# lambdaclass/lambdaworks_cairo_prover

Hardware: AMD Instinct MI355X
Metric: stark252_ntt_field_ops_per_s (higher is better)
Workload: dtype u256 mod p (8 x u32 Montgomery limbs); 1 GPU; Stark252 forward NTT 2^22, natural order in/out, one vector per GPU (BASELINE configs[1]); log_n=22, parallelism=replicas x1 (column sharding, no collective), self_warmup_steps=930

## Files before the change

include/stark252_hip.h:

```cpp
#ifndef STARK252_HIP_H
#define STARK252_HIP_H
#include <stddef.h>
#include <stdint.h>

#ifdef __cplusplus
extern "C" {
#endif

enum {
    SP_OK = 0,
    SP_E_INVALID_ARG = -1,
    SP_E_NO_DEVICE = -2,
    SP_E_HIP = -3,
    SP_E_ALLOC = -4,
    SP_E_STATE = -5,
    SP_E_ZERO_INVERSE = -6,
    SP_E_UNSUPPORTED = -7,
    SP_E_PROGRAM = -8
};

typedef enum { SP_FE_MONT_LIMBS = 0, SP_FE_CANON_BE = 1 } sp_fe_encoding;

typedef struct {
    uint8_t blowup_factor;
// ... 16 lines not shown

typedef int (*sp_allgather_fn)(void* user, const void* send_dev, void* recv_dev, uint64_t bytes_per_rank);

const char* sp_version(void);
#define SP_ABI_VERSION 7
int sp_abi_version(void);
uint64_t sp_air_desc_size(void);
const char* sp_last_error(void);
int sp_device_count(int* count_out);
int sp_host_cpus(int* count_out);
int sp_host_cpu_budget(int* budget_out, int* ranks_out);
int sp_host_bind_to_device(int device, int* node_out);

int sp_ctx_create(sp_ctx** ctx_out, const sp_config* cfg);
void sp_ctx_destroy(sp_ctx* ctx);

int sp_set_collective(sp_ctx* ctx, int world, int rank, sp_allgather_fn fn, void* user);
int sp_comm_unique_id(uint8_t id_out[128]);
int sp_comm_init_rccl(sp_ctx* ctx, const uint8_t id[128], int world, int rank);
typedef int (*sp_allgather_async_fn)(void* user, const void* send_dev, void* recv_dev, uint64_t bytes_per_rank, void* hip_stream);
int sp_set_collective_async(sp_ctx* ctx, sp_allgather_async_fn fn);
int sp_comm_init_null(sp_ctx* ctx, int world, int rank);
typedef int (*sp_alltoall_fn)(void* user, const void* send_dev, void* recv_dev, uint64_t bytes_per_pair);
int sp_set_alltoall(sp_ctx* ctx, sp_alltoall_fn fn);
typedef int (*sp_alltoall_async_fn)(void* user, const void* send_dev, void* recv_dev, uint64_t bytes_per_pair, void* hip_stream);
int sp_set_alltoall_async(sp_ctx* ctx, sp_alltoall_async_fn fn);
int sp_comm_stats(sp_ctx* ctx, uint64_t out[6]);
int sp_comm_time_ms(sp_ctx* ctx, double out[2]);
int sp_comm_selftest(sp_ctx* ctx, uint64_t bytes_per_block);
#define SP_LINK_MEASURED_MARGIN 1.25
int sp_comm_measure(sp_ctx* ctx, uint64_t bytes_per_rank, double out[6]);
int sp_model_shard_interpolation(double link_gbs_per_direction, uint32_t groups, uint32_t log2_rows);
enum { SP_OPT_FRI_SHARD_MIN_LOG = 1, SP_OPT_SHARD_INTERPOLATION = 2, SP_OPT_UPLOAD_THREADS = 3, SP_OPT_MERKLE_BACKEND = 4, SP_OPT_MERKLE_ONE_COLUMN_ROWS = 5,
       SP_OPT_DEVICE_TRACE = 6, SP_OPT_LINK_GBS = 7, SP_OPT_HOST_RANKS = 8 };
enum { SP_MERKLE_KECCAK256 = 0, SP_MERKLE_POSEIDON = 1 };
int sp_set_option(sp_ctx* ctx, int key, int64_t value);


int sp_ntt(sp_ctx* ctx, uint8_t* data, uint64_t n, int inverse, const uint8_t* coset);

int sp_ntt_dev(sp_ctx* ctx, void* data_dev, uint64_t n, uint32_t batch, int inverse, const uint8_t* coset);

int sp_lde(sp_ctx* ctx, const uint8_t* coeffs, uint64_t n, uint32_t cols, uint32_t blowup, const uint8_t* coset,
           uint8_t* out);

int sp_merkle_build(sp_ctx* ctx, const uint8_t* leaves, uint64_t n_leaves, uint32_t fe_per_leaf,
                    uint8_t root_out[32], uint8_t* nodes_out);

int sp_merkle_build_dev(sp_ctx* ctx, const void* cols_dev, uint64_t n_leaves, uint32_t fe_per_leaf, uint64_t col_stride,
                        void* nodes_dev);

int sp_batch_inverse(sp_ctx* ctx, uint8_t* data, uint64_t n);
int sp_fe_mul(sp_ctx* ctx, const uint8_t* a, const uint8_t* b, uint64_t n, uint8_t* out);

int sp_fe_to_device(int fe_encoding, const uint8_t* in, uint64_t n, uint8_t* out_device_layout);
int sp_fe_from_device(int fe_encoding, const uint8_t* in_device_layout, uint64_t n, uint8_t* out);

int sp_sync(sp_ctx* ctx);
int sp_last_kernel_ms(sp_ctx* ctx, float* ms_out);
int sp_timer_start(sp_ctx* ctx);
int sp_timer_stop(sp_ctx* ctx, float* ms_out);

typedef struct {
    uint8_t pc_init[32], ap_init[32], fp_init[32], pc_final[32], ap_final[32];
    uint16_t range_check_min, range_check_max;
    uint32_t n_segments;
    const uint8_t* segment_types;
// ... 244 lines not shown
```

lambdaworks_cairo_prover_amd/api.py:

```python
import ctypes
from dataclasses import dataclass

import numpy as np

from . import _lib
from ._lib import (SP_FE_CANON_BE, SP_FE_MONT_LIMBS, CairoPublicInputsC, ConfigC, ProofOptionsC, SpError, check)

__all__ = ["ProofOptions", "Context", "CairoRun", "generate_prover_args_fibonacci", "SpError", "P", "felts_to_bytes",
           "bytes_to_felts", "SP_FE_CANON_BE", "SP_FE_MONT_LIMBS"]

P = 2**251 + 17 * 2**192 + 1


def felts_to_bytes(values):
    return np.frombuffer(b"".join(int(v).to_bytes(32, "big") for v in values), dtype=np.uint8).reshape(-1, 32).copy()


def bytes_to_felts(arr):
    b = np.ascontiguousarray(arr, dtype=np.uint8).tobytes()
    return [int.from_bytes(b[i:i + 32], "big") for i in range(0, len(b), 32)]


@dataclass
class ProofOptions:
# ... 719 lines not shown
    check(self._lib.sp_comm_selftest(self._h, ctypes.c_uint64(bytes_per_block)))


def _ctx_comm_measure(self, bytes_per_rank=64 << 20):
    out = (ctypes.c_double * 6)()
    check(self._lib.sp_comm_measure(self._h, ctypes.c_uint64(int(bytes_per_rank)), out))
    return {"allgather_ms": out[0], "allgather_gbs_per_link": out[1], "alltoall_ms": out[2], "alltoall_gbs_per_link": out[3],
            "bytes_per_rank": int(out[4]), "world": int(out[5])}


LINK_MEASURED_MARGIN = 1.25


def model_shard_interpolation(link_gbs, groups, log2_rows):
    lib = _lib.load()
    lib.sp_model_shard_interpolation.argtypes = [ctypes.c_double, ctypes.c_uint32, ctypes.c_uint32]
    return int(lib.sp_model_shard_interpolation(float(link_gbs), int(groups), int(log2_rows)))


def _ctx_comm_time_ms(self):
    out = (ctypes.c_double * 2)()
    check(self._lib.sp_comm_time_ms(self._h, out))
    return out[0], out[1]


def _ctx_comm_stats(self):
    out = (ctypes.c_uint64 * 6)()
    check(self._lib.sp_comm_stats(self._h, out))
    return {"world": out[0], "allgather_calls": out[1], "allgather_bytes": out[2], "alltoall_calls": out[3],
            "alltoall_bytes": out[4], "received_bytes": out[5]}


SP_OPT_FRI_SHARD_MIN_LOG, SP_OPT_SHARD_INTERPOLATION, SP_OPT_UPLOAD_THREADS, SP_OPT_MERKLE_BACKEND, SP_OPT_MERKLE_ONE_COLUMN_ROWS, SP_OPT_DEVICE_TRACE, SP_OPT_LINK_GBS, SP_OPT_HOST_RANKS = 1, 2, 3, 4, 5, 6, 7, 8
SP_MERKLE_KECCAK256, SP_MERKLE_POSEIDON = 0, 1
SP_PREWARM_KERNELS, SP_PREWARM_CLOCKS, SP_PREWARM_HOST_ROWS, SP_PREWARM_ALL = 1, 2, 4, 7


def _ctx_set_option(self, key, value):
    check(self._lib.sp_set_option(self._h, int(key), ctypes.c_int64(int(value))))


def _ctx_init_rccl(self, group=None):
    import torch
    import torch.distributed as dist
    world, rank = dist.get_world_size(group), dist.get_rank(group)
    idb = (ctypes.c_uint8 * 128)()
    if rank == 0:
        check(self._lib.sp_comm_unique_id(idb))
    obj = [bytes(idb)]
    dist.broadcast_object_list(obj, src=0, group=group)
    check(self._lib.sp_comm_init_rccl(self._h, obj[0], world, rank))


Context.set_collective = _ctx_set_collective
Context.init_rccl = _ctx_init_rccl
Context.init_null = _ctx_init_null
Context.set_collective_async = _ctx_set_collective_async
Context.comm_stats = _ctx_comm_stats
Context.comm_selftest = _ctx_comm_selftest
Context.comm_measure = _ctx_comm_measure
Context.comm_time_ms = _ctx_comm_time_ms
Context.set_option = _ctx_set_option
__all__ += ["cairo_verify", "proof_file_bytes", "proof_file_verify", "StagedAllGather", "StagedAsyncAllGather", "shard_global_index", "interleave_shards",
            "SP_OPT_FRI_SHARD_MIN_LOG", "SP_OPT_SHARD_INTERPOLATION", "SP_OPT_UPLOAD_THREADS", "SP_OPT_MERKLE_BACKEND", "SP_OPT_MERKLE_ONE_COLUMN_ROWS", "SP_OPT_DEVICE_TRACE", "SP_OPT_LINK_GBS", "SP_OPT_HOST_RANKS", "host_cpu_budget", "last_error", "model_shard_interpolation",
            "SP_MERKLE_KECCAK256", "SP_MERKLE_POSEIDON", "poseidon_host", "host_bind_to_device",
            "SP_PREWARM_KERNELS", "SP_PREWARM_CLOCKS", "SP_PREWARM_HOST_ROWS", "SP_PREWARM_ALL"]
```

lambdaworks_cairo_prover_amd/csrc/capi_dev.cpp:

```cpp
#include "ctx.h"
#include "cairo_host.h"
#include <rccl/rccl.h>
#include <chrono>
#include <cstdlib>
#include <algorithm>
#include <cstring>
#include <vector>

namespace sp { int air_periodic_tables(hipStream_t st, NttEngine& ntt, fe* vals, fe* ws, fe* tab, uint32_t cnt, uint32_t logp, uint32_t logn, uint32_t logb, const fe& h); }
namespace sp { int air_stride_class_tables(hipStream_t st, NttEngine& ntt, fe* u, fe* z, uint32_t logs, uint32_t offset, uint32_t logn, uint32_t logb, const fe& h); }
using namespace sp;

namespace {
struct DevBuf {
    void* p = nullptr;
    ~DevBuf() { if (p) (void)hipFree(p); }
    int alloc(size_t bytes) {
        if (hipMalloc(&p, bytes ? bytes : 1) != hipSuccess) { sp_set_error("hipMalloc failed (" + std::to_string(bytes) + " bytes)"); p = nullptr; return SP_E_ALLOC; }
        return SP_OK;
    }
    template <class T> T* as() { return reinterpret_cast<T*>(p); }
};
}

// ... 101 lines not shown
int sp_set_option(sp_ctx* c, int key, int64_t value) {
    if (!c) return SP_E_INVALID_ARG;
    switch (key) {
        case SP_OPT_FRI_SHARD_MIN_LOG:
            if (value < 1 || value > 40) return SP_E_INVALID_ARG;
            c->opt_fri_shard_min_log = (uint32_t)value;
            break;
        case SP_OPT_SHARD_INTERPOLATION:
            if (value < 0 || value > 2) return SP_E_INVALID_ARG;
            c->opt_shard_interpolation = (int)value;
            break;
        case SP_OPT_LINK_GBS:
            if (value < 1 || value > 10000) return SP_E_INVALID_ARG;
            c->opt_link_gbs = (double)value;
            c->opt_link_gbs_explicit = true;
            break;
        case SP_OPT_UPLOAD_THREADS:
            if (value < 1 || value > 128) return SP_E_INVALID_ARG;
            c->opt_upload_threads = (uint32_t)value;
            break;
        case SP_OPT_MERKLE_BACKEND:
            if (value != SP_MERKLE_KECCAK256 && value != SP_MERKLE_POSEIDON) return SP_E_INVALID_ARG;
            c->opt_merkle_backend = (int)value;
            break;
        case SP_OPT_HOST_RANKS:
            if (value < 0 || value > 1024) return SP_E_INVALID_ARG;
            sp::set_host_ranks((unsigned)value);
            return SP_OK;
        case SP_OPT_DEVICE_TRACE:
            c->opt_device_trace = value != 0;
            return SP_OK;
        case SP_OPT_MERKLE_ONE_COLUMN_ROWS:
            c->opt_merkle_one_column_rows = value != 0;
            return SP_OK;
        default: sp_set_error("sp_set_option: unknown key"); return SP_E_INVALID_ARG;
    }
    delete c->prover_state_deleter_holder;
    c->prover_state_deleter_holder = nullptr;
    return SP_OK;
}

namespace {
struct RcclComm : public sp_deletable {
    ncclComm_t comm = nullptr;
    hipStream_t stream = nullptr;
    int world = 1;
    ~RcclComm() override { if (comm) (void)ncclCommDestroy(comm); }
};
int rccl_allgather(void* user, const void* send, void* recv, uint64_t bytes) {
    RcclComm* rc = static_cast<RcclComm*>(user);
    if (ncclAllGather(send, recv, bytes, ncclUint8, rc->comm, rc->stream) != ncclSuccess) return -1;
    if (hipStreamSynchronize(rc->stream) != hipSuccess) return -2;
    return 0;
}
int rccl_allgather_async(void* user, const void* send, void* recv, uint64_t bytes, void* stream) {
    RcclComm* rc = static_cast<RcclComm*>(user);
    return ncclAllGather(send, recv, bytes, ncclUint8, rc->comm, static_cast<hipStream_t>(stream)) == ncclSuccess ? 0 : -1;
}
int rccl_alltoall_async(void* user, const void* send, void* recv, uint64_t bytes, void* stream) {
    RcclComm* rc = static_cast<RcclComm*>(user);
    hipStream_t st = static_cast<hipStream_t>(stream);
    const uint8_t* s = static_cast<const uint8_t*>(send);
    uint8_t* r = static_cast<uint8_t*>(recv);
    if (ncclGroupStart() != ncclSuccess) return -1;
    int rcode = 0;
    for (int peer = 0; peer < rc->world && rcode == 0; ++peer) {
// ... 524 lines not shown
```

lambdaworks_cairo_prover_amd/csrc/ntt.h:

```cpp
#pragma once
#include "common.h"
#include <map>
#include <vector>

namespace sp {

constexpr int NTT_TILE_LOG = 10;
constexpr int NTT_THREADS = 256;
constexpr int NTT_MAX_CONTIG_LOG = NTT_TILE_LOG;
constexpr int NTT_STRIDED_G_LOG = 2;
constexpr int NTT_MAX_STRIDED_LOG = NTT_TILE_LOG - NTT_STRIDED_G_LOG;

struct NttPassArgs {
    const fe* src;
    fe* dst;
    uint64_t src_vec_stride, dst_vec_stride;
    const fe* small_tw;
    const fe* big_tw;
    const fe* post_table;
    const fe* scalar;
    uint32_t logM;
    uint32_t logL;
    uint32_t s, r, g;
    uint32_t log_expand;
    uint32_t tw_shift, tw_low;
    uint32_t coset_count, shard_log;
    uint64_t src_coset_stride, dst_coset_stride;
    uint32_t weak_out;
    uint32_t stage_tw;
    uint32_t radix4;
    uint32_t batch;
    uint32_t xcd_map;
};

enum NttLoadMode { NTT_LOAD_INPLACE = 0, NTT_LOAD_GATHER_BITREV = 1, NTT_LOAD_EXPAND = 2 };
enum NttStoreMode { NTT_STORE_INPLACE = 0, NTT_STORE_SCATTER_BITREV = 1 };

class NttEngine {
  public:
    explicit NttEngine(hipStream_t stream) : stream_(stream) {}
    ~NttEngine();
    int roots(int k, const fe** out);
    int stage_tables(int k, const fe** out);
    int inv_roots_small(int k, const fe** out);

    int dit_bitrev_to_natural(fe* data, int k, uint32_t batch, uint64_t stride);
    int dif_natural_to_bitrev_inverse(fe* data, int k, uint32_t batch, uint64_t stride, const fe* post_table, const fe* src = nullptr);
    int forward_natural(const fe* src, fe* dst, int k, uint32_t batch, uint64_t src_stride, uint64_t dst_stride, fe* final_dst = nullptr);
    int inverse_natural(fe* data, fe* tmp, int k, uint32_t batch, uint64_t stride);
    int lde_from_bitrev(const fe* coeffs, fe* dst, int k, int logb, uint32_t batch, uint64_t src_stride, uint64_t dst_stride,
                        int shard_log = 0, int shard_rank = 0);
    int lde_coset_major(const fe* coeffs, fe* dst, int k, int logb, uint32_t batch, uint64_t src_stride, uint64_t dst_stride,
                        int shard_log = 0, int shard_rank = 0);

    int scale_by_powers(fe* data, uint64_t n, uint32_t batch, uint64_t stride, const fe& base, const fe* c);

    hipStream_t stream() const { return stream_; }

  private:
    int launch_pass(bool dif, int load_mode, int store_mode, const NttPassArgs& a, uint32_t batch);
    hipStream_t stream_;
    int transform_twiddles(int k, NttPassArgs* a);
    std::map<int, fe*> roots_;
    std::vector<fe*> pyramids_;
    int pyramid_log_ = -1;
    std::map<int, fe*> inv_small_;
    fe* d_scalar_ = nullptr;
};

fe host_primitive_root(int k);

}
```

lambdaworks_cairo_prover_amd/csrc/ntt.hip:

```cpp
#include "ntt.h"
#include <algorithm>

#ifndef SP_NTT_STAGE_TW
#define SP_NTT_STAGE_TW 1
#endif

namespace sp {

__device__ __forceinline__ fe ld_fe(const fe* p) {
    const uint4* q = reinterpret_cast<const uint4*>(p);
    uint4 lo = q[0], hi = q[1];
    fe r;
    r.v[0] = lo.x; r.v[1] = lo.y; r.v[2] = lo.z; r.v[3] = lo.w;
    r.v[4] = hi.x; r.v[5] = hi.y; r.v[6] = hi.z; r.v[7] = hi.w;
    return r;
}
__device__ __forceinline__ void st_fe(fe* p, const fe& a) {
    uint4* q = reinterpret_cast<uint4*>(p);
    q[0] = make_uint4(a.v[0], a.v[1], a.v[2], a.v[3]);
    q[1] = make_uint4(a.v[4], a.v[5], a.v[6], a.v[7]);
}
__device__ __forceinline__ fe lds_ld(const uint4* lo, const uint4* hi, uint32_t i) {
    uint4 a = lo[i], b = hi[i];
    fe r;
    r.v[0] = a.x; r.v[1] = a.y; r.v[2] = a.z; r.v[3] = a.w;
    r.v[4] = b.x; r.v[5] = b.y; r.v[6] = b.z; r.v[7] = b.w;
    return r;
}
__device__ __forceinline__ void lds_st(uint4* lo, uint4* hi, uint32_t i, const fe& a) {
    lo[i] = make_uint4(a.v[0], a.v[1], a.v[2], a.v[3]);
    hi[i] = make_uint4(a.v[4], a.v[5], a.v[6], a.v[7]);
}
__device__ __forceinline__ uint32_t bitrev(uint32_t x, uint32_t bits) { return bits ? (__brev(x) >> (32 - bits)) : 0u; }

template <bool DIF, int LOADM, int STOREM, bool CONTIG, bool GTW>
__global__ void __launch_bounds__(NTT_THREADS) ntt_pass_kernel(NttPassArgs a) {
    extern __shared__ __attribute__((aligned(16))) uint4 smem[];
#ifndef SP_NTT_PRIO
#define SP_NTT_PRIO 1
#endif
    if (SP_NTT_PRIO & 1) __builtin_amdgcn_s_setprio(3);
    const uint32_t r = a.r, g = a.g;
    const uint32_t s = a.s;
    const uint32_t R = 1u << r, G = 1u << g, TILE = R << g;
    constexpr bool GLOBAL_TW = GTW;
    static_assert(GTW || CONTIG, "strided passes stage the twiddles of their own butterflies");
    uint4* Llo = smem;
    uint4* Lhi = smem + TILE;
    uint4* Twl = smem + 2 * TILE;
    uint4* Twh = Twl + (GLOBAL_TW ? (CONTIG ? R : (a.radix4 ? (TILE >> 2) : (TILE >> 1))) : (R >> 1));
    const uint32_t tid = threadIdx.x;
    uint32_t tile, vec;
    if (a.xcd_map) {
        const uint32_t xcd = blockIdx.x & 7u, slot = blockIdx.x >> 3;
        const uint32_t tg = slot / a.batch;
        vec = slot - tg * a.batch;
        tile = (tg << 3) | xcd;
    } else {
        tile = blockIdx.x / a.batch;
        vec = blockIdx.x - tile * a.batch;
    }
    uint32_t tw_low = a.tw_low;
    const fe* src;
    fe* dst;
    if (a.coset_count) {
        const uint32_t v = vec / a.coset_count, cl = vec - v * a.coset_count;
        src = a.src + (uint64_t)v * a.src_vec_stride + (uint64_t)cl * a.src_coset_stride;
        dst = a.dst + (uint64_t)v * a.dst_vec_stride + (uint64_t)cl * a.dst_coset_stride;
        tw_low |= cl << a.shard_log;
    } else {
        src = a.src + (uint64_t)vec * a.src_vec_stride;
        dst = a.dst + (uint64_t)vec * a.dst_vec_stride;
    }
    const uint32_t logM = a.logM;
    const uint32_t logL = a.logL;
    const uint32_t sg = s + a.tw_shift;

    uint32_t lo0 = 0, hi = 0;
    if (!CONTIG) {
        uint32_t lo_tiles = 1u << (s - g);
        lo0 = (tile & (lo_tiles - 1)) << g;
        hi = tile >> (s - g);
    }
    auto global_tw = [&](uint32_t jm1, uint32_t i, uint32_t gl) -> fe {
        const uint32_t col = ((lo0 + gl) << a.tw_shift) | tw_low;
        const uint32_t x = (i << sg) + col, h = 1u << (sg + jm1);
        const bool pyr = SP_NTT_STAGE_TW && a.stage_tw;
        const uint32_t sh = pyr ? 0u : logM - sg - jm1 - 1u, off = pyr ? h : 0u;
        if (!DIF) return ld_fe(a.big_tw + off + (x << sh));
        if (x == 0) return fe_neg_one();
        return ld_fe(a.big_tw + off + ((h - x) << sh));
    };
    constexpr int BPT = (1 << (NTT_TILE_LOG - 1)) / NTT_THREADS;
    fe tw_last[(GLOBAL_TW && !CONTIG) ? BPT : 1];
    fe tw_pen;
    if (GLOBAL_TW && CONTIG) {
        for (uint32_t x = tid; x + 1 < R; x += NTT_THREADS) {
            const uint32_t y = x + 1u, jm1 = 31u - __clz(y);
            lds_st(Twl, Twh, x, global_tw(jm1, y - (1u << jm1), 0u));
        }
    } else if (GLOBAL_TW) {
        if (r >= 1) {
#pragma unroll
            for (int q = 0; q < BPT; ++q) {
                const uint32_t b = tid + q * (a.radix4 ? (TILE >> 2) : (uint32_t)NTT_THREADS);
                if (b < (TILE >> 1)) tw_last[q] = global_tw(r - 1, b >> g, b & (G - 1));
            }
            if (a.radix4 && r >= 2 && tid < (TILE >> 2)) tw_pen = global_tw(r - 2, tid >> g, tid & (G - 1));
            const uint32_t cnt = (a.radix4 ? (TILE >> 2) : (TILE >> 1)) - G;
            fe tmp[BPT];
#pragma unroll
            for (int q = 0; q < BPT; ++q) {
                const uint32_t x = tid + q * NTT_THREADS;
                if (x < cnt) {
                    const uint32_t y = (x >> g) + 1u;
                    const uint32_t jm1 = 31u - __clz(y);
                    tmp[q] = global_tw(jm1, y - (1u << jm1), x & (G - 1));
                }
            }
#pragma unroll
            for (int q = 0; q < BPT; ++q) {
                const uint32_t x = tid + q * NTT_THREADS;
                if (x < cnt) lds_st(Twl, Twh, x, tmp[q]);
            }
        }
    } else {
        for (uint32_t i = tid; i < (R >> 1); i += NTT_THREADS) lds_st(Twl, Twh, i, ld_fe(a.small_tw + i));
    }
    auto position = [&](uint32_t t, uint32_t gl) -> uint32_t {
        if (CONTIG) {
            if (LOADM == NTT_LOAD_GATHER_BITREV || STOREM == NTT_STORE_SCATTER_BITREV)
                return (bitrev((tile << g) + gl, logL - r) << r) + t;
            return (tile << (r + g)) + (gl << r) + t;
        }
        return (hi << (s + r)) + (t << s) + lo0 + gl;
    };
    auto lidx = [&](uint32_t t, uint32_t gl) -> uint32_t { return CONTIG ? (gl << r) + t : (t << g) + gl; };

    constexpr int LU = 4;
    for (uint32_t e0 = tid; e0 < TILE; e0 += NTT_THREADS * LU) {
        fe xs[LU];
        uint32_t li[LU];
#pragma unroll
        for (int q = 0; q < LU; ++q) {
            const uint32_t e = e0 + q * NTT_THREADS;
            if (e >= TILE) continue;
            uint32_t t, gl;
            if (CONTIG && LOADM == NTT_LOAD_INPLACE) {
                t = e & (R - 1); gl = e >> r;
                xs[q] = ld_fe(src + position(t, gl));
            } else if (CONTIG) {
                gl = e & (G - 1); t = e >> g;
                uint32_t sidx = (bitrev(t, r) << (logL - r)) + (tile << g) + gl;
                xs[q] = ld_fe(src + sidx);
            } else {
                gl = e & (G - 1); t = e >> g;
                uint32_t pos = position(t, gl);
                if (LOADM == NTT_LOAD_EXPAND) xs[q] = ld_fe(src + (pos >> s));
                else xs[q] = ld_fe(src + pos);
            }
            li[q] = lidx(t, gl);
        }
#pragma unroll
        for (int q = 0; q < LU; ++q)
            if (e0 + q * NTT_THREADS < TILE) lds_st(Llo, Lhi, li[q], xs[q]);
    }
    if (SP_NTT_PRIO & 1) __builtin_amdgcn_s_setprio(0);
    __syncthreads();

// ... 114 lines not shown
                    const uint32_t q = half;
                    st_fe(dst + position(t0, gl), a.weak_out ? fe_reduce_lazy_2p(y0) : fe_canonical_lazy(y0));
                    st_fe(dst + position(t0 + q, gl), a.weak_out ? fe_reduce_lazy_2p(y1) : fe_canonical_lazy(y1));
                    st_fe(dst + position(t0 + 2 * q, gl), a.weak_out ? fe_reduce_lazy_2p(y2) : fe_canonical_lazy(y2));
                    st_fe(dst + position(t0 + 3 * q, gl), a.weak_out ? fe_reduce_lazy_2p(y3) : fe_canonical_lazy(y3));
                } else {
                    lds_st(Llo, Lhi, l0, y0); lds_st(Llo, Lhi, l2, y2); lds_st(Llo, Lhi, l1, y1); lds_st(Llo, Lhi, l3, y3);
                }
            }
            if (j + 1 != r || a.radix4 != 1) __syncthreads();
        }
        if (a.radix4 == 1) return;
    }

    if (SP_NTT_PRIO & 2) __builtin_amdgcn_s_setprio(3);
    fe scal;
    const bool has_scalar = a.scalar != nullptr;
    if (has_scalar) scal = ld_fe(a.scalar);
    for (uint32_t e = tid; e < TILE; e += NTT_THREADS) {
        uint32_t t, gl;
        if (CONTIG && STOREM == NTT_STORE_INPLACE) { t = e & (R - 1); gl = e >> r; }
        else { gl = e & (G - 1); t = e >> g; }
        fe x = lds_ld(Llo, Lhi, lidx(t, gl));
        uint32_t pos = position(t, gl);
        uint32_t didx = pos;
        if (CONTIG && STOREM == NTT_STORE_SCATTER_BITREV) didx = (bitrev(t, r) << (logL - r)) + (tile << g) + gl;
        if (DIF && a.post_table) x = fe_mul_lazy(x, ld_fe(a.post_table + didx));
        if (has_scalar) x = fe_mul_lazy(x, scal);
        x = a.weak_out ? fe_reduce_lazy_2p(x) : fe_canonical_lazy(x);
        st_fe(dst + didx, x);
    }
}

struct RootGenArgs { fe pw[32]; };
__global__ void gen_roots_kernel(fe* table, uint32_t count, uint32_t bits, RootGenArgs args) {
    uint32_t e = blockIdx.x * blockDim.x + threadIdx.x;
    if (e >= count) return;
    fe acc = fe_one();
    for (uint32_t i = 0; i < bits; ++i)
        if ((e >> i) & 1) acc = fe_mul(acc, args.pw[i]);
    st_fe(table + e, acc);
}

struct PowArgs { fe pw[40]; fe c; uint32_t has_c; };
__global__ void scale_powers_kernel(fe* data, uint64_t n, uint64_t stride, PowArgs args) {
    uint64_t i = (uint64_t)blockIdx.x * blockDim.x + threadIdx.x;
    if (i >= n) return;
    fe acc = args.has_c ? args.c : fe_one();
    for (uint32_t b = 0; b < 40; ++b)
        if ((i >> b) & 1) acc = fe_mul(acc, args.pw[b]);
    fe* p = data + (uint64_t)blockIdx.y * stride + i;
    st_fe(p, fe_mul(ld_fe(p), acc));
}

static const uint8_t TWO_ADIC_ROOT_BE[32] = {0x00, 0x52, 0x82, 0xdb, 0x87, 0x52, 0x9c, 0xfa, 0x3f, 0x04, 0x64, 0x51, 0x9c, 0x8b, 0x0f, 0xa5,
                                             0xad, 0x18, 0x71, 0x48, 0xe1, 0x1a, 0x61, 0x61, 0x60, 0x70, 0x02, 0x4f, 0x42, 0xf8, 0xef, 0x94};

fe host_primitive_root(int k) {
    fe w = fe_from_bytes_be(TWO_ADIC_ROOT_BE);
    for (int i = k; i < 192; ++i) w = fe_sqr(w);
    return w;
}

NttEngine::~NttEngine() {
    for (auto& kv : roots_) (void)hipFree(kv.second);
    for (fe* p : pyramids_) (void)hipFree(p);
// ... 59 lines not shown
    if (!pyr) SP_TRY(roots(k, &a->big_tw));
    return SP_OK;
}
int NttEngine::inv_roots_small(int k, const fe** out) {
    auto it = inv_small_.find(k);
    if (it == inv_small_.end()) {
        fe* d = nullptr;
        uint32_t count = k == 0 ? 1u : (1u << (k - 1));
        SP_TRY(gen_table(stream_, fe_inv(host_primitive_root(k)), k, count, &d));
        it = inv_small_.emplace(k, d).first;
    }
    *out = it->second;
    return SP_OK;
}

template <bool DIF, int LM, int SM, bool CONTIG, bool GTW>
static int launch_t(hipStream_t st, const NttPassArgs& a, uint32_t batch) {
    uint32_t tile_log = a.r + a.g;
    uint32_t tiles = 1u << (a.logL - tile_log);
    size_t lds = ((size_t)2 << tile_log) * sizeof(uint4) + ((size_t)1 << a.r) * sizeof(uint4);
    if (!CONTIG) lds = ((size_t)3 << tile_log) * sizeof(uint4);
    else if (GTW) lds = ((size_t)2 << tile_log) * sizeof(uint4) + ((size_t)2 << a.r) * sizeof(uint4);
    NttPassArgs b = a;
    b.batch = batch;
    b.xcd_map = (tiles % 8 == 0) ? 1u : 0u;
    b.radix4 = (a.r >= 2 && (1u << tile_log) == 4u * NTT_THREADS) ? 1u : 0u;
    if (!CONTIG && b.radix4) lds = ((size_t)5 << (tile_log - 1)) * sizeof(uint4);
    if ((uint64_t)tiles * batch >= (1ull << 31)) { sp_set_error("ntt: batch too large for one launch"); return SP_E_INVALID_ARG; }
    hipLaunchKernelGGL((ntt_pass_kernel<DIF, LM, SM, CONTIG, GTW>), dim3(tiles * batch), dim3(NTT_THREADS), lds, st, b);
    SP_HIP_CHECK(hipGetLastError());
    return SP_OK;
}

int NttEngine::launch_pass(bool dif, int lm, int sm, const NttPassArgs& a, uint32_t batch) {
    bool contig = a.s == 0 && lm != NTT_LOAD_EXPAND;
    if (!dif) {
        if (contig && a.coset_count) return launch_t<false, NTT_LOAD_INPLACE, NTT_STORE_INPLACE, true, true>(stream_, a, batch);
        if (contig && lm == NTT_LOAD_INPLACE) return launch_t<false, NTT_LOAD_INPLACE, NTT_STORE_INPLACE, true, false>(stream_, a, batch);
        if (contig && lm == NTT_LOAD_GATHER_BITREV) return launch_t<false, NTT_LOAD_GATHER_BITREV, NTT_STORE_INPLACE, true, false>(stream_, a, batch);
        if (!contig && lm == NTT_LOAD_INPLACE) return launch_t<false, NTT_LOAD_INPLACE, NTT_STORE_INPLACE, false, true>(stream_, a, batch);
        if (!contig && lm == NTT_LOAD_EXPAND) return launch_t<false, NTT_LOAD_EXPAND, NTT_STORE_INPLACE, false, true>(stream_, a, batch);
    } else {
        if (contig && sm == NTT_STORE_INPLACE) return launch_t<true, NTT_LOAD_INPLACE, NTT_STORE_INPLACE, true, false>(stream_, a, batch);
        if (contig && sm == NTT_STORE_SCATTER_BITREV) return launch_t<true, NTT_LOAD_INPLACE, NTT_STORE_SCATTER_BITREV, true, false>(stream_, a, batch);
        if (!contig) return launch_t<true, NTT_LOAD_INPLACE, NTT_STORE_INPLACE, false, true>(stream_, a, batch);
    }
    sp_set_error("ntt: unsupported pass mode");
    return SP_E_UNSUPPORTED;
}

struct PassGeom { int s, r, g; };
static std::vector<PassGeom> geometry(int k, int first_stride_log, int first_contig_max, uint64_t footprint) {
    const int min_tile_log = footprint > (64ull << 20) ? 10 : 9;
    std::vector<PassGeom> out;
    int s = first_stride_log;
    int rem = k - first_stride_log;
    if (rem <= 0) return out;
    if (s == 0) {
        int r1 = std::min(rem, first_contig_max);
        int g = std::min(NTT_TILE_LOG - r1, k - r1);
        out.push_back({0, r1, g});
        s = r1; rem -= r1;
    }
    if (rem > 0) {
        int np = (rem + NTT_MAX_STRIDED_LOG - 1) / NTT_MAX_STRIDED_LOG;
        std::vector<int> takes;
        for (int i = 0, left = rem; i < np; ++i) { int take = (left + (np - i) - 1) / (np - i); takes.push_back(take); left -= take; }
#ifndef SP_NTT_EVEN_SPLIT
#define SP_NTT_EVEN_SPLIT 1
#endif
        if (SP_NTT_EVEN_SPLIT)
            for (size_t i = 0; i < takes.size(); ++i)
                for (size_t j = i + 1; j < takes.size(); ++j)
                    if ((takes[i] & 1) && (takes[j] & 1) && takes[i] + 1 <= NTT_MAX_STRIDED_LOG && takes[j] >= 3) { takes[i] += 1; takes[j] -= 1; }
        for (int take : takes) {
            int g = std::min(std::max(NTT_STRIDED_G_LOG, min_tile_log - take), s);
            out.push_back({s, take, g});
            s += take;
        }
    }
    return out;
}

int NttEngine::dit_bitrev_to_natural(fe* data, int k, uint32_t batch, uint64_t stride) {
    if (k == 0) return SP_OK;
    NttPassArgs tw{};
    SP_TRY(transform_twiddles(k, &tw));
    std::vector<PassGeom> geo = geometry(k, 0, NTT_MAX_CONTIG_LOG, ((uint64_t)batch << k) * sizeof(fe));
    for (size_t i = 0; i < geo.size(); ++i) {
        const PassGeom& p = geo[i];
        NttPassArgs a{};
        a.src = data; a.dst = data; a.src_vec_stride = a.dst_vec_stride = stride;
        SP_TRY(roots(p.r, &a.small_tw));
        a.big_tw = tw.big_tw; a.stage_tw = tw.stage_tw; a.logM = k; a.logL = k; a.s = p.s; a.r = p.r; a.g = p.g;
        a.weak_out = i + 1 < geo.size();
        SP_TRY(launch_pass(false, NTT_LOAD_INPLACE, NTT_STORE_INPLACE, a, batch));
    }
    return SP_OK;
}

int NttEngine::dif_natural_to_bitrev_inverse(fe* data, int k, uint32_t batch, uint64_t stride, const fe* post_table, const fe* src) {
    NttPassArgs tw{};
    SP_TRY(transform_twiddles(k, &tw));
    constexpr int contig_cap = 7;
    std::vector<PassGeom> geo = geometry(k, 0, k <= NTT_TILE_LOG ? NTT_TILE_LOG : contig_cap, ((uint64_t)batch << k) * sizeof(fe));
    if (geo.empty()) geo.push_back({0, 0, 0});
    for (size_t i = geo.size(); i-- > 0;) {
        const PassGeom& p = geo[i];
        NttPassArgs a{};
        a.src = (src && i + 1 == geo.size()) ? src : data;
        a.dst = data; a.src_vec_stride = a.dst_vec_stride = stride;
        SP_TRY(inv_roots_small(p.r, &a.small_tw));
        a.big_tw = tw.big_tw; a.stage_tw = tw.stage_tw; a.logM = k; a.logL = k; a.s = p.s; a.r = p.r; a.g = p.g;
        a.weak_out = i != 0;
        if (i == 0) a.post_table = post_table;
        SP_TRY(launch_pass(true, NTT_LOAD_INPLACE, NTT_STORE_INPLACE, a, batch));
    }
    return SP_OK;
}

int NttEngine::forward_natural(const fe* src, fe* dst, int k, uint32_t batch, uint64_t ss, uint64_t ds, fe* final_dst) {
    NttPassArgs tw{};
    SP_TRY(transform_twiddles(k, &tw));
    std::vector<PassGeom> geo = geometry(k, 0, k <= NTT_TILE_LOG ? NTT_TILE_LOG : NTT_TILE_LOG - NTT_STRIDED_G_LOG, ((uint64_t)batch << k) * sizeof(fe));
    if (geo.empty()) geo.push_back({0, 0, 0});
    bool first = true;
    const fe* cur = src; uint64_t cur_stride = ss;
    size_t pi = 0;
    for (const PassGeom& p : geo) {
// ... 54 lines not shown
        return dit_bitrev_to_natural(dst, k, batch, ds);
    }
    const fe* big = nullptr;
    SP_TRY(roots(K, &big));
    std::vector<PassGeom> geo = geometry(K, logb, NTT_MAX_CONTIG_LOG, ((uint64_t)batch << (K - shard_log)) * sizeof(fe));
    if (geo.empty()) {
        geo.push_back({logb, 0, std::min(logb, NTT_STRIDED_G_LOG)});
    }
    bool first = true;
    size_t pi = 0;
    for (const PassGeom& p : geo) {
        NttPassArgs a{};
        a.src = first ? coeffs : dst; a.dst = dst;
        a.src_vec_stride = first ? ss : ds; a.dst_vec_stride = ds;
        a.weak_out = ++pi < geo.size();
        SP_TRY(roots(p.r, &a.small_tw));
        a.big_tw = big; a.logM = K; a.logL = (uint32_t)(K - shard_log); a.s = (uint32_t)(p.s - shard_log); a.r = p.r; a.log_expand = logb;
        a.tw_shift = (uint32_t)shard_log; a.tw_low = (uint32_t)shard_rank;
        a.g = (uint32_t)std::min<int>(p.g, p.s - shard_log);
        SP_TRY(launch_pass(false, first ? NTT_LOAD_EXPAND : NTT_LOAD_INPLACE, NTT_STORE_INPLACE, a, batch));
        first = false;
    }
    return SP_OK;
}

int NttEngine::lde_coset_major(const fe* coeffs, fe* dst, int k, int logb, uint32_t batch, uint64_t ss, uint64_t ds, int shard_log, int shard_rank) {
    const int K = k + logb;
    if (shard_log < 0 || shard_log > logb) { sp_set_error("lde: more shards than cosets"); return SP_E_INVALID_ARG; }
    const uint32_t b_loc = 1u << (logb - shard_log);
    const uint64_t n = 1ull << k;
    const fe* big = nullptr;
    SP_TRY(roots(K, &big));
    constexpr int contig_cap = NTT_TILE_LOG - NTT_STRIDED_G_LOG;
    std::vector<PassGeom> geo = geometry(k, 0, k <= NTT_TILE_LOG ? NTT_TILE_LOG : contig_cap, ((uint64_t)batch * b_loc << k) * sizeof(fe));
    if (geo.empty()) geo.push_back({0, 0, 0});
    bool first = true;
    size_t pi = 0;
    for (const PassGeom& p : geo) {
        NttPassArgs a{};
        a.src = first ? coeffs : dst; a.dst = dst;
        a.src_vec_stride = first ? ss : ds; a.dst_vec_stride = ds;
        a.coset_count = b_loc; a.src_coset_stride = first ? 0 : n; a.dst_coset_stride = n;
        a.weak_out = ++pi < geo.size();
        a.big_tw = big; a.logM = K; a.logL = (uint32_t)k; a.s = p.s; a.r = p.r; a.g = p.g;
        a.tw_shift = (uint32_t)logb; a.tw_low = (uint32_t)shard_rank; a.shard_log = (uint32_t)shard_log;
        SP_TRY(launch_pass(false, NTT_LOAD_INPLACE, NTT_STORE_INPLACE, a, batch * b_loc));
        first = false;
    }
    return SP_OK;
}

int NttEngine::scale_by_powers(fe* data, uint64_t n, uint32_t batch, uint64_t stride, const fe& base, const fe* c) {
    PowArgs args;
    fe cur = base;
    for (int i = 0; i < 40; ++i) { args.pw[i] = cur; cur = fe_sqr(cur); }
    args.has_c = c ? 1 : 0;
    args.c = c ? *c : fe_one();
    dim3 grid((unsigned)((n + 255) / 256), batch);
    hipLaunchKernelGGL(scale_powers_kernel, grid, dim3(256), 0, stream_, data, n, stride, args);
    SP_HIP_CHECK(hipGetLastError());
    return SP_OK;
}

}
```

Before: 143.3 billion butterflies/s.

## Add register-tiled two-pass NTT kernel for large transforms

Adds a register-tiled DIT pass kernel: each thread holds 8 field elements in registers and does three radix-2 stages per round, exchanging through a swizzled LDS buffer between rounds. Large NTTs (footprint over 64 MiB, k up to 20) are split into exactly two such passes, the aim being fewer global-memory round trips than the existing multi-pass geometry. Address and twiddle logic is factored into a shared PassAddr helper. The cost is many LDS exchanges and syncs per pass, plus global twiddle loads for the upper stages.

```diff
diff --git a/include/stark252_hip.h b/include/stark252_hip.h
--- a/include/stark252_hip.h
+++ b/include/stark252_hip.h
@@ -72,7 +72,7 @@
 int sp_comm_measure(sp_ctx* ctx, uint64_t bytes_per_rank, double out[6]);
 int sp_model_shard_interpolation(double link_gbs_per_direction, uint32_t groups, uint32_t log2_rows);
 enum { SP_OPT_FRI_SHARD_MIN_LOG = 1, SP_OPT_SHARD_INTERPOLATION = 2, SP_OPT_UPLOAD_THREADS = 3, SP_OPT_MERKLE_BACKEND = 4, SP_OPT_MERKLE_ONE_COLUMN_ROWS = 5,
-       SP_OPT_DEVICE_TRACE = 6, SP_OPT_LINK_GBS = 7, SP_OPT_HOST_RANKS = 8 };
+       SP_OPT_DEVICE_TRACE = 6, SP_OPT_LINK_GBS = 7, SP_OPT_HOST_RANKS = 8, SP_OPT_NTT_TWO_PASS = 9 };
 enum { SP_MERKLE_KECCAK256 = 0, SP_MERKLE_POSEIDON = 1 };
 int sp_set_option(sp_ctx* ctx, int key, int64_t value);
 
diff --git a/lambdaworks_cairo_prover_amd/api.py b/lambdaworks_cairo_prover_amd/api.py
--- a/lambdaworks_cairo_prover_amd/api.py
+++ b/lambdaworks_cairo_prover_amd/api.py
@@ -775,6 +775,7 @@
 
 
 SP_OPT_FRI_SHARD_MIN_LOG, SP_OPT_SHARD_INTERPOLATION, SP_OPT_UPLOAD_THREADS, SP_OPT_MERKLE_BACKEND, SP_OPT_MERKLE_ONE_COLUMN_ROWS, SP_OPT_DEVICE_TRACE, SP_OPT_LINK_GBS, SP_OPT_HOST_RANKS = 1, 2, 3, 4, 5, 6, 7, 8
+SP_OPT_NTT_TWO_PASS = 9
 SP_MERKLE_KECCAK256, SP_MERKLE_POSEIDON = 0, 1
 SP_PREWARM_KERNELS, SP_PREWARM_CLOCKS, SP_PREWARM_HOST_ROWS, SP_PREWARM_ALL = 1, 2, 4, 7
 
@@ -805,6 +806,6 @@
 Context.comm_time_ms = _ctx_comm_time_ms
 Context.set_option = _ctx_set_option
 __all__ += ["cairo_verify", "proof_file_bytes", "proof_file_verify", "StagedAllGather", "StagedAsyncAllGather", "shard_global_index", "interleave_shards",
-            "SP_OPT_FRI_SHARD_MIN_LOG", "SP_OPT_SHARD_INTERPOLATION", "SP_OPT_UPLOAD_THREADS", "SP_OPT_MERKLE_BACKEND", "SP_OPT_MERKLE_ONE_COLUMN_ROWS", "SP_OPT_DEVICE_TRACE", "SP_OPT_LINK_GBS", "SP_OPT_HOST_RANKS", "host_cpu_budget", "last_error", "model_shard_interpolation",
+            "SP_OPT_FRI_SHARD_MIN_LOG", "SP_OPT_SHARD_INTERPOLATION", "SP_OPT_UPLOAD_THREADS", "SP_OPT_MERKLE_BACKEND", "SP_OPT_MERKLE_ONE_COLUMN_ROWS", "SP_OPT_DEVICE_TRACE", "SP_OPT_LINK_GBS", "SP_OPT_HOST_RANKS", "SP_OPT_NTT_TWO_PASS", "host_cpu_budget", "last_error", "model_shard_interpolation",
             "SP_MERKLE_KECCAK256", "SP_MERKLE_POSEIDON", "poseidon_host", "host_bind_to_device",
             "SP_PREWARM_KERNELS", "SP_PREWARM_CLOCKS", "SP_PREWARM_HOST_ROWS", "SP_PREWARM_ALL"]
diff --git a/lambdaworks_cairo_prover_amd/csrc/capi_dev.cpp b/lambdaworks_cairo_prover_amd/csrc/capi_dev.cpp
--- a/lambdaworks_cairo_prover_amd/csrc/capi_dev.cpp
+++ b/lambdaworks_cairo_prover_amd/csrc/capi_dev.cpp
@@ -157,6 +157,10 @@
             return SP_OK;
         case SP_OPT_MERKLE_ONE_COLUMN_ROWS:
             c->opt_merkle_one_column_rows = value != 0;
+            return SP_OK;
+        case SP_OPT_NTT_TWO_PASS:
+            if (value < 0 || value > 2) return SP_E_INVALID_ARG;
+            c->ntt->set_two_pass((int)value);
             return SP_OK;
         default: sp_set_error("sp_set_option: unknown key"); return SP_E_INVALID_ARG;
     }
diff --git a/lambdaworks_cairo_prover_amd/csrc/ntt.h b/lambdaworks_cairo_prover_amd/csrc/ntt.h
--- a/lambdaworks_cairo_prover_amd/csrc/ntt.h
+++ b/lambdaworks_cairo_prover_amd/csrc/ntt.h
@@ -10,6 +10,10 @@
 constexpr int NTT_MAX_CONTIG_LOG = NTT_TILE_LOG;
 constexpr int NTT_STRIDED_G_LOG = 2;
 constexpr int NTT_MAX_STRIDED_LOG = NTT_TILE_LOG - NTT_STRIDED_G_LOG;
+
+constexpr int NTT_RT_LOG = 12;
+constexpr int NTT_RT_THREADS = 512;
+constexpr int NTT_RT_MAX_STAGES = 10;
 
 struct NttPassArgs {
     const fe* src;
@@ -55,11 +59,16 @@
 
     int scale_by_powers(fe* data, uint64_t n, uint32_t batch, uint64_t stride, const fe& base, const fe* c);
 
+    void set_two_pass(int mode) { two_pass_ = mode; }
+
     hipStream_t stream() const { return stream_; }
 
   private:
     int launch_pass(bool dif, int load_mode, int store_mode, const NttPassArgs& a, uint32_t batch);
+    int launch_regtile(const NttPassArgs& a, uint32_t batch);
     hipStream_t stream_;
+    int two_pass_ = 2;
+    bool regtile_ready_[2] = {false, false};
     int transform_twiddles(int k, NttPassArgs* a);
     std::map<int, fe*> roots_;
     std::vector<fe*> pyramids_;
diff --git a/lambdaworks_cairo_prover_amd/csrc/ntt.hip b/lambdaworks_cairo_prover_amd/csrc/ntt.hip
--- a/lambdaworks_cairo_prover_amd/csrc/ntt.hip
+++ b/lambdaworks_cairo_prover_amd/csrc/ntt.hip
@@ -32,6 +32,59 @@
     hi[i] = make_uint4(a.v[4], a.v[5], a.v[6], a.v[7]);
 }
 __device__ __forceinline__ uint32_t bitrev(uint32_t x, uint32_t bits) { return bits ? (__brev(x) >> (32 - bits)) : 0u; }
+
+template <bool DIF, bool CONTIG, bool BITREV>
+struct PassAddr {
+    const NttPassArgs& a;
+    uint32_t tile, tw_low, lo0 = 0, hi = 0;
+    uint32_t sg;
+    const fe* src;
+    fe* dst;
+    __device__ __forceinline__ explicit PassAddr(const NttPassArgs& args) : a(args) {
+        uint32_t vec;
+        if (a.xcd_map) {
+            const uint32_t xcd = blockIdx.x & 7u, slot = blockIdx.x >> 3;
+            const uint32_t tg = slot / a.batch;
+            vec = slot - tg * a.batch;
+            tile = (tg << 3) | xcd;
+        } else {
+            tile = blockIdx.x / a.batch;
+            vec = blockIdx.x - tile * a.batch;
+        }
+        tw_low = a.tw_low;
+        if (a.coset_count) {
+            const uint32_t v = vec / a.coset_count, cl = vec - v * a.coset_count;
+            src = a.src + (uint64_t)v * a.src_vec_stride + (uint64_t)cl * a.src_coset_stride;
+            dst = a.dst + (uint64_t)v * a.dst_vec_stride + (uint64_t)cl * a.dst_coset_stride;
+            tw_low |= cl << a.shard_log;
+        } else {
+            src = a.src + (uint64_t)vec * a.src_vec_stride;
+            dst = a.dst + (uint64_t)vec * a.dst_vec_stride;
+        }
+        sg = a.s + a.tw_shift;
+        if (!CONTIG) {
+            const uint32_t lo_tiles = 1u << (a.s - a.g);
+            lo0 = (tile & (lo_tiles - 1)) << a.g;
+            hi = tile >> (a.s - a.g);
+        }
+    }
+    __device__ __forceinline__ fe global_tw(uint32_t jm1, uint32_t i, uint32_t gl) const {
+        const uint32_t col = ((lo0 + gl) << a.tw_shift) | tw_low;
+        const uint32_t x = (i << sg) + col, h = 1u << (sg + jm1);
+        const bool pyr = SP_NTT_STAGE_TW && a.stage_tw;
+        const uint32_t sh = pyr ? 0u : a.logM - sg - jm1 - 1u, off = pyr ? h : 0u;
+        if (!DIF) return ld_fe(a.big_tw + off + (x << sh));
+        if (x == 0) return fe_neg_one();
+        return ld_fe(a.big_tw + off + ((h - x) << sh));
+    }
+    __device__ __forceinline__ uint32_t position(uint32_t t, uint32_t gl) const {
+        if (CONTIG) {
+            if (BITREV) return (bitrev((tile << a.g) + gl, a.logL - a.r) << a.r) + t;
+            return (tile << (a.r + a.g)) + (gl << a.r) + t;
+        }
+        return (hi << (a.s + a.r)) + (t << a.s) + lo0 + gl;
+    }
+};
 
 template <bool DIF, int LOADM, int STOREM, bool CONTIG, bool GTW>
 __global__ void __launch_bounds__(NTT_THREADS) ntt_pass_kernel(NttPassArgs a) {
@@ -50,47 +103,12 @@
     uint4* Twl = smem + 2 * TILE;
     uint4* Twh = Twl + (GLOBAL_TW ? (CONTIG ? R : (a.radix4 ? (TILE >> 2) : (TILE >> 1))) : (R >> 1));
     const uint32_t tid = threadIdx.x;
-    uint32_t tile, vec;
-    if (a.xcd_map) {
-        const uint32_t xcd = blockIdx.x & 7u, slot = blockIdx.x >> 3;
-        const uint32_t tg = slot / a.batch;
-        vec = slot - tg * a.batch;
-        tile = (tg << 3) | xcd;
-    } else {
-        tile = blockIdx.x / a.batch;
-        vec = blockIdx.x - tile * a.batch;
-    }
-    uint32_t tw_low = a.tw_low;
-    const fe* src;
-    fe* dst;
-    if (a.coset_count) {
-        const uint32_t v = vec / a.coset_count, cl = vec - v * a.coset_count;
-        src = a.src + (uint64_t)v * a.src_vec_stride + (uint64_t)cl * a.src_coset_stride;
-        dst = a.dst + (uint64_t)v * a.dst_vec_stride + (uint64_t)cl * a.dst_coset_stride;
-        tw_low |= cl << a.shard_log;
-    } else {
-        src = a.src + (uint64_t)vec * a.src_vec_stride;
-        dst = a.dst + (uint64_t)vec * a.dst_vec_stride;
-    }
-    const uint32_t logM = a.logM;
+    const PassAddr<DIF, CONTIG, LOADM == NTT_LOAD_GATHER_BITREV || STOREM == NTT_STORE_SCATTER_BITREV> ad(a);
+    const uint32_t tile = ad.tile;
+    const fe* src = ad.src;
+    fe* dst = ad.dst;
     const uint32_t logL = a.logL;
-    const uint32_t sg = s + a.tw_shift;
-
-    uint32_t lo0 = 0, hi = 0;
-    if (!CONTIG) {
-        uint32_t lo_tiles = 1u << (s - g);
-        lo0 = (tile & (lo_tiles - 1)) << g;
-        hi = tile >> (s - g);
-    }
-    auto global_tw = [&](uint32_t jm1, uint32_t i, uint32_t gl) -> fe {
-        const uint32_t col = ((lo0 + gl) << a.tw_shift) | tw_low;
-        const uint32_t x = (i << sg) + col, h = 1u << (sg + jm1);
-        const bool pyr = SP_NTT_STAGE_TW && a.stage_tw;
-        const uint32_t sh = pyr ? 0u : logM - sg - jm1 - 1u, off = pyr ? h : 0u;
-        if (!DIF) return ld_fe(a.big_tw + off + (x << sh));
-        if (x == 0) return fe_neg_one();
-        return ld_fe(a.big_tw + off + ((h - x) << sh));
-    };
+    auto global_tw = [&](uint32_t jm1, uint32_t i, uint32_t gl) -> fe { return ad.global_tw(jm1, i, gl); };
     constexpr int BPT = (1 << (NTT_TILE_LOG - 1)) / NTT_THREADS;
     fe tw_last[(GLOBAL_TW && !CONTIG) ? BPT : 1];
     fe tw_pen;
@@ -127,14 +145,7 @@
     } else {
         for (uint32_t i = tid; i < (R >> 1); i += NTT_THREADS) lds_st(Twl, Twh, i, ld_fe(a.small_tw + i));
     }
-    auto position = [&](uint32_t t, uint32_t gl) -> uint32_t {
-        if (CONTIG) {
-            if (LOADM == NTT_LOAD_GATHER_BITREV || STOREM == NTT_STORE_SCATTER_BITREV)
-                return (bitrev((tile << g) + gl, logL - r) << r) + t;
-            return (tile << (r + g)) + (gl << r) + t;
-        }
-        return (hi << (s + r)) + (t << s) + lo0 + gl;
-    };
+    auto position = [&](uint32_t t, uint32_t gl) -> uint32_t { return ad.position(t, gl); };
     auto lidx = [&](uint32_t t, uint32_t gl) -> uint32_t { return CONTIG ? (gl << r) + t : (t << g) + gl; };
 
     constexpr int LU = 4;
@@ -315,6 +326,105 @@
     }
 }
 
+constexpr int NTT_RT_TW = 512;
+constexpr size_t NTT_RT_LDS = (((size_t)1 << NTT_RT_LOG) + 2 * NTT_RT_TW) * sizeof(uint4);
+
+__device__ __forceinline__ uint32_t rt_elem(uint32_t u, uint32_t B, uint32_t m) { return ((u >> B) << (B + 3)) | (m << B) | (u & ((1u << B) - 1u)); }
+__device__ __forceinline__ uint32_t rt_slot(uint32_t e) { return e ^ (((e >> 4) & 3u) << 1) ^ (((e >> 6) & 1u) * 9u); }
+__device__ __forceinline__ void rt_butterfly(fe& u, fe& v, const fe& w) {
+    const fe t = fe_mul_lazy(v, w);
+    v = fe_sub_add_2p(u, t);
+    u = fe_add_raw(u, t);
+}
+
+template <bool CONTIG>
+__global__ void __launch_bounds__(NTT_RT_THREADS) __attribute__((amdgpu_waves_per_eu(4, 4))) ntt_regtile_pass_kernel(NttPassArgs a) {
+    extern __shared__ __attribute__((aligned(16))) uint4 smem[];
+    uint4* X = smem;
+    uint4* Twl = smem + (1u << NTT_RT_LOG);
+    uint4* Twh = Twl + NTT_RT_TW;
+    const PassAddr<false, CONTIG, false> ad(a);
+    const uint32_t r = a.r, g = a.g, u = threadIdx.x;
+    const uint32_t gt = CONTIG ? 0u : g;
+    const uint32_t tbit = CONTIG ? 0u : g;
+    const uint32_t jl = min(r, 9u - gt);
+    {
+        const uint32_t cnt = ((1u << jl) - 1u) << gt;
+        if (u < cnt) {
+            const uint32_t y = (u >> gt) + 1u, jm1 = 31u - __clz(y);
+            lds_st(Twl, Twh, u, ad.global_tw(jm1, y - (1u << jm1), u & ((1u << gt) - 1u)));
+        }
+    }
+    auto row = [&](uint32_t e) -> uint32_t { return CONTIG ? (e & ((1u << r) - 1u)) : (e >> g); };
+    auto col = [&](uint32_t e) -> uint32_t { return CONTIG ? (e >> r) : (e & ((1u << g) - 1u)); };
+
+    fe x[8];
+    uint32_t Bcur = CONTIG ? 9u : g;
+#pragma unroll
+    for (int m = 0; m < 8; ++m) {
+        const uint32_t e = rt_elem(u, Bcur, m);
+        x[m] = ld_fe(ad.src + ad.position(row(e), col(e)));
+    }
+    __syncthreads();
+
+    auto exchange = [&](uint32_t Bo, uint32_t Bn) {
+        uint32_t so[8], sn[8];
+#pragma unroll
+        for (int m = 0; m < 8; ++m) { so[m] = rt_slot(rt_elem(u, Bo, m)); sn[m] = rt_slot(rt_elem(u, Bn, m)); }
+#pragma unroll
+        for (int m = 0; m < 8; ++m) X[so[m]] = make_uint4(x[m].v[0], x[m].v[1], x[m].v[2], x[m].v[3]);
+        __syncthreads();
+#pragma unroll
+        for (int m = 0; m < 8; ++m) { const uint4 q = X[sn[m]]; x[m].v[0] = q.x; x[m].v[1] = q.y; x[m].v[2] = q.z; x[m].v[3] = q.w; }
+        __syncthreads();
+#pragma unroll
+        for (int m = 0; m < 8; ++m) X[so[m]] = make_uint4(x[m].v[4], x[m].v[5], x[m].v[6], x[m].v[7]);
+        __syncthreads();
+#pragma unroll
+        for (int m = 0; m < 8; ++m) { const uint4 q = X[sn[m]]; x[m].v[4] = q.x; x[m].v[5] = q.y; x[m].v[6] = q.z; x[m].v[7] = q.w; }
+        __syncthreads();
+    };
+    if (CONTIG) { exchange(Bcur, 0u); Bcur = 0u; }
+
+    for (uint32_t done = 0, b = 0;;) {
+        const uint32_t e0 = rt_elem(u, Bcur, 0u);
+        const uint32_t i0 = row(e0) & ((1u << b) - 1u), gl = CONTIG ? 0u : col(e0), step = 1u << b;
+        auto tw = [&](uint32_t jm1, uint32_t i) -> fe {
+            if (jm1 < jl) return lds_ld(Twl, Twh, (((1u << jm1) - 1u + i) << gt) + gl);
+            return ad.global_tw(jm1, i, gl);
+        };
+        if (done <= b) {
+            const fe w = tw(b, i0);
+            rt_butterfly(x[0], x[1], w); rt_butterfly(x[2], x[3], w); rt_butterfly(x[4], x[5], w); rt_butterfly(x[6], x[7], w);
+            __builtin_amdgcn_sched_barrier(0);
+        }
+        if (done <= b + 1u) {
+            fe w = tw(b + 1u, i0);
+            rt_butterfly(x[0], x[2], w); rt_butterfly(x[4], x[6], w);
+            __builtin_amdgcn_sched_barrier(0);
+            w = tw(b + 1u, i0 + step);
+            rt_butterfly(x[1], x[3], w); rt_butterfly(x[5], x[7], w);
+            __builtin_amdgcn_sched_barrier(0);
+        }
+#pragma unroll
+        for (int m = 0; m < 4; ++m) {
+            rt_butterfly(x[m], x[m + 4], tw(b + 2u, i0 + m * step));
+            __builtin_amdgcn_sched_barrier(0);
+        }
+        done = b + 3u;
+        if (done >= r) break;
+        b = (done + 3u <= r) ? done : r - 3u;
+        exchange(Bcur, b + tbit);
+        Bcur = b + tbit;
+    }
+
+#pragma unroll
+    for (int m = 0; m < 8; ++m) {
+        const uint32_t e = rt_elem(u, Bcur, m);
+        st_fe(ad.dst + ad.position(row(e), col(e)), a.weak_out ? fe_reduce_lazy_2p(x[m]) : fe_canonical_lazy(x[m]));
+    }
+}
+
 struct RootGenArgs { fe pw[32]; };
 __global__ void gen_roots_kernel(fe* table, uint32_t count, uint32_t bits, RootGenArgs args) {
     uint32_t e = blockIdx.x * blockDim.x + threadIdx.x;
@@ -440,6 +550,30 @@
     return SP_OK;
 }
 
+int NttEngine::launch_regtile(const NttPassArgs& a, uint32_t batch) {
+    if (a.r < 6 || a.r > 10 || a.r + a.g != (uint32_t)NTT_RT_LOG || a.logL < (uint32_t)NTT_RT_LOG || a.s + a.r > a.logL || (a.s != 0 && a.s < a.g) ||
+        a.s + a.tw_shift + a.r > a.logM) {
+        sp_set_error("ntt: shape outside the register-tile passes (6 <= r <= 10, r + g = 12)");
+        return SP_E_INVALID_ARG;
+    }
+    const bool contig = a.s == 0;
+    const uint32_t tiles = 1u << (a.logL - NTT_RT_LOG);
+    if ((uint64_t)tiles * batch >= (1ull << 31)) { sp_set_error("ntt: batch too large for one launch"); return SP_E_INVALID_ARG; }
+    NttPassArgs b = a;
+    b.batch = batch;
+    b.xcd_map = (tiles % 8 == 0) ? 1u : 0u;
+    static_assert(NTT_RT_LDS <= 81920, "two work-groups per CU");
+    if (!regtile_ready_[contig]) {
+        const void* fn = contig ? reinterpret_cast<const void*>(&ntt_regtile_pass_kernel<true>) : reinterpret_cast<const void*>(&ntt_regtile_pass_kernel<false>);
+        SP_HIP_CHECK(hipFuncSetAttribute(fn, hipFuncAttributeMaxDynamicSharedMemorySize, (int)NTT_RT_LDS));
+        regtile_ready_[contig] = true;
+    }
+    if (contig) hipLaunchKernelGGL((ntt_regtile_pass_kernel<true>), dim3(tiles * batch), dim3(NTT_RT_THREADS), NTT_RT_LDS, stream_, b);
+    else hipLaunchKernelGGL((ntt_regtile_pass_kernel<false>), dim3(tiles * batch), dim3(NTT_RT_THREADS), NTT_RT_LDS, stream_, b);
+    SP_HIP_CHECK(hipGetLastError());
+    return SP_OK;
+}
+
 int NttEngine::launch_pass(bool dif, int lm, int sm, const NttPassArgs& a, uint32_t batch) {
     bool contig = a.s == 0 && lm != NTT_LOAD_EXPAND;
     if (!dif) {
@@ -457,10 +591,17 @@
     return SP_E_UNSUPPORTED;
 }
 
-struct PassGeom { int s, r, g; };
-static std::vector<PassGeom> geometry(int k, int first_stride_log, int first_contig_max, uint64_t footprint) {
-    const int min_tile_log = footprint > (64ull << 20) ? 10 : 9;
+struct PassGeom { int s, r, g; bool regtile = false; };
+static std::vector<PassGeom> geometry(int k, int first_stride_log, int first_contig_max, uint64_t footprint, int two_pass = 0) {
+    const bool large = footprint > (64ull << 20);
+    const int min_tile_log = large ? 10 : 9;
     std::vector<PassGeom> out;
+    if (first_stride_log == 0 && k >= NTT_RT_LOG && k <= 2 * NTT_RT_MAX_STAGES && (two_pass == 1 || (two_pass == 2 && large))) {
+        const int r1 = (k + 1) / 2, r2 = k / 2;
+        out.push_back({0, r1, NTT_RT_LOG - r1, true});
+        out.push_back({r1, r2, NTT_RT_LOG - r2, true});
+        return out;
+    }
     int s = first_stride_log;
     int rem = k - first_stride_log;
     if (rem <= 0) return out;
@@ -494,7 +635,7 @@
     if (k == 0) return SP_OK;
     NttPassArgs tw{};
     SP_TRY(transform_twiddles(k, &tw));
-    std::vector<PassGeom> geo = geometry(k, 0, NTT_MAX_CONTIG_LOG, ((uint64_t)batch << k) * sizeof(fe));
+    std::vector<PassGeom> geo = geometry(k, 0, NTT_MAX_CONTIG_LOG, ((uint64_t)batch << k) * sizeof(fe), two_pass_);
     for (size_t i = 0; i < geo.size(); ++i) {
         const PassGeom& p = geo[i];
         NttPassArgs a{};
@@ -502,7 +643,8 @@
         SP_TRY(roots(p.r, &a.small_tw));
         a.big_tw = tw.big_tw; a.stage_tw = tw.stage_tw; a.logM = k; a.logL = k; a.s = p.s; a.r = p.r; a.g = p.g;
         a.weak_out = i + 1 < geo.size();
-        SP_TRY(launch_pass(false, NTT_LOAD_INPLACE, NTT_STORE_INPLACE, a, batch));
+        if (p.regtile) SP_TRY(launch_regtile(a, batch));
+        else SP_TRY(launch_pass(false, NTT_LOAD_INPLACE, NTT_STORE_INPLACE, a, batch));
     }
     return SP_OK;
 }
@@ -623,7 +765,7 @@
     const fe* big = nullptr;
     SP_TRY(roots(K, &big));
     constexpr int contig_cap = NTT_TILE_LOG - NTT_STRIDED_G_LOG;
-    std::vector<PassGeom> geo = geometry(k, 0, k <= NTT_TILE_LOG ? NTT_TILE_LOG : contig_cap, ((uint64_t)batch * b_loc << k) * sizeof(fe));
+    std::vector<PassGeom> geo = geometry(k, 0, k <= NTT_TILE_LOG ? NTT_TILE_LOG : contig_cap, ((uint64_t)batch * b_loc << k) * sizeof(fe), two_pass_);
     if (geo.empty()) geo.push_back({0, 0, 0});
     bool first = true;
     size_t pi = 0;
@@ -635,7 +777,8 @@
         a.weak_out = ++pi < geo.size();
         a.big_tw = big; a.logM = K; a.logL = (uint32_t)k; a.s = p.s; a.r = p.r; a.g = p.g;
         a.tw_shift = (uint32_t)logb; a.tw_low = (uint32_t)shard_rank; a.shard_log = (uint32_t)shard_log;
-        SP_TRY(launch_pass(false, NTT_LOAD_INPLACE, NTT_STORE_INPLACE, a, batch * b_loc));
+        if (p.regtile) SP_TRY(launch_regtile(a, batch * b_loc));
+        else SP_TRY(launch_pass(false, NTT_LOAD_INPLACE, NTT_STORE_INPLACE, a, batch * b_loc));
         first = false;
     }
     return SP_OK;
```

Result: no change. 142.1 billion butterflies/s (-0.9%).
